# VISION-SJTU/UniDefense

Measured on AMD Instinct MI355X. Metric: images/sec fwd+bwd (256x256, EffNet-b4), higher is better.
Workload: dtype f32

## Files before the change

include/unidefense_hip.h:

```cpp
#ifndef UNIDEFENSE_HIP_H
#define UNIDEFENSE_HIP_H
#include <stdint.h>

#ifdef __cplusplus
extern "C" {
#endif

#define UD_EINVAL (-1000)

typedef void* ud_stream_t;

typedef struct {
    int N, Hin, Win, Cin, Hout, Wout, KH, KW, stride, pad_t, pad_l, transposed;
} ud_conv_geom;

typedef struct {
    const float* A; const float* B; float* C;
    int M, N, K;
    long lda, ldb, ldc;
    int a_mode, b_mode, out_mode, split_k;
    int batch; long strideA, strideB, strideC;
    ud_conv_geom g;
    double* stat_sum; double* stat_sumsq;
    int half_mask;
    int tile_cfg;
    long slice_stride;
} ud_gemm_desc;
int ud_gemm(const ud_gemm_desc* d, ud_stream_t stream);
int ud_sum_slices(const float* ws, float* out, int slices, long total, long slice_stride, int accumulate,
                  ud_stream_t stream);
int ud_gemm_stats_slots(const ud_gemm_desc* d);
int ud_stat_slots_fold(const double* slot_sum, const double* slot_sumsq, int slots, int N, double* acc_sum,
                       double* acc_sumsq, ud_stream_t stream);
int ud_gemm_set_path(int path);
int ud_gemm_get_path(void);
int ud_gemm_query_path(const ud_gemm_desc* d);

typedef struct {
    const uint16_t* A; const uint16_t* B; float* C;
    int M, N, K;
    long a_panel, a_plane, b_panel, b_plane;
    int a_npanel, b_npanel;
    long ldc;
    int a_mode, b_mode, out_mode, split_k;
    double* stat_sum; double* stat_sumsq;
    int tile_cfg;
    long slice_stride;
    int prec;
    const float* a_inv_scale; const float* b_inv_scale;
    int a_scale_stride, b_scale_stride;
    int c_half;
} ud_gemm_p3_desc;
int ud_gemm_p3(const ud_gemm_p3_desc* d, ud_stream_t stream);
int ud_gemm_p3_pair(const ud_gemm_p3_desc* nn, const ud_gemm_p3_desc* tn, ud_stream_t stream);
int ud_planes_from_half(const void* x, long R, int C, long ld, uint16_t* planes, long panel_stride, float* inv_scale,
                        ud_stream_t stream);
int ud_split_planes(const float* x, long R, int C, long ld, uint16_t* planes, long panel_stride, long plane_stride,
                    ud_stream_t stream);
int ud_split_planes_h2(const float* x, long R, int C, long ld, uint16_t* planes, long panel_stride, long plane_stride,
                       float* inv_scale, ud_stream_t stream);
int ud_absmax(const float* x, long R, int C, long ld, uint32_t* absmax, ud_stream_t stream);
int ud_split_planes_h2t(const float* x, long R, int C, long ld, uint16_t* planes, long panel_stride, long plane_stride,
                        const uint32_t* absmax, float* inv_scale, ud_stream_t stream);
typedef struct {
    const float* x; uint16_t* out; float* inv_scale;
    long R, ld, panel, plane;
    int C, amax_block0, amax_blocks, split_block0, split_bx, pad_;
} ud_split_item;
int ud_split_planes_h2t_multi(const ud_split_item* items_dev, int n, uint32_t* slots, int amax_blocks_total,
                              int split_blocks_total, ud_stream_t stream);

int ud_im2col_planes(const float* x, const ud_conv_geom* g, uint16_t* planes, long panel_stride, long plane_stride,
                     const uint32_t* absmax, float* inv_scale, ud_stream_t stream);
int ud_col2im(const float* dcol, const ud_conv_geom* g, float* dx, ud_stream_t stream);

typedef struct {
    const float* src;
    float* dst;
    int A, B, KH, KW, mode, block0;
} ud_layout_item;
int ud_weight_layouts_multi(const ud_layout_item* items_dev, int n, int blocks_total, ud_stream_t stream);

int ud_reduce_ws_doubles(int G, int R, int C);
int ud_norm_stats(const float* x, int G, int R, int C, float eps, double* ws, float* mean, float* invstd,
                  float* var_out, float momentum, float* running_mean, float* running_var, ud_stream_t stream);
int ud_syncbn_combine(const float* gathered, int world, int C, long rows_per_rank, float eps, float momentum,
                      float* running_mean, float* running_var, float* mean, float* invstd, ud_stream_t stream);
int ud_norm_apply_fwd(const float* x, int G, int R, int C, const float* mean, const float* invstd,
                      const float* gamma, const float* beta, int act, float* y, ud_stream_t stream);
int ud_norm_bwd(const float* x, const float* dy, int G, int R, int C, const float* mean, const float* invstd,
                const float* gamma, const float* beta, int act, double* ws, float* s1, float* s2, float* dgamma,
                float* dbeta, float* dx, ud_stream_t stream);
int ud_norm_bwd_apply(const float* x, const float* dy, int G, int R, int C, const float* mean,
                      const float* invstd, const float* gamma, const float* beta, const float* s1,
                      const float* s2, float inv_count, int act, float* dx, ud_stream_t stream);
int ud_group_colsum(const float* x, int G, int R, int C, float scale, double* ws, float* out, ud_stream_t stream);
int ud_group_coldot(const float* a, const float* b, int G, int R, int C, float scale, double* ws, float* out,
                    ud_stream_t stream);
int ud_bcast_rows(const float* g, float scale, float* out, int N, int HW, int C, ud_stream_t stream);

int ud_dwconv_fwd(const void* x, const float* wt, void* y, int N, int H, int W, int C, int Ho, int Wo, int K,
    int stride, int pad_t, int pad_l, int f16, ud_stream_t stream);
int ud_dwconv_bwd_data(const void* dy, const float* wt, const void* add, void* dx, int N, int H, int W, int C,
    int Ho, int Wo, int K, int stride, int pad_t, int pad_l, int f16, ud_stream_t stream);
int ud_dwconv_bwd_weight_parts(int C, int chunks);
int ud_dw_weights_tapmajor(const void* table, int layers, long max_elems, float* dst, ud_stream_t stream);
int ud_dwconv_bwd_weight(const float* x, const float* dy, float* dwt, float* part, int chunks, int N,
// ... 543 lines not shown
```

unidefense_amd/csrc/gemm_p3.hip:

```cpp
#include "gemm_internal.h"
#include "ud_common.h"

#include <algorithm>
#include <type_traits>

namespace {

constexpr int NT = 512;
constexpr int BK = 32;
constexpr int BM = 128, BN = 128;
constexpr int PLANE_IMG = 128 * 64;

template <int PREC> struct Cfg {
    static constexpr int NPL = PREC;
    static constexpr int OP_IMG = NPL * PLANE_IMG;
    static constexpr int STAGE = 2 * OP_IMG;
    static constexpr int NSTAGE = PREC == 3 ? 3 : 4;
    static constexpr int PT = 4 * NPL;
    static constexpr int NTERM = PREC == 3 ? 6 : PREC == 2 ? 3 : 1;
};

typedef __bf16 bf16x8 __attribute__((ext_vector_type(8)));
typedef _Float16 f16x8 __attribute__((ext_vector_type(8)));
typedef short s16x4 __attribute__((ext_vector_type(4)));
typedef short s16x8 __attribute__((ext_vector_type(8)));
typedef __attribute__((address_space(3))) char lds_char;

__device__ __forceinline__ void dma_piece(unsigned voff, unsigned lds_dst, const char* gbase) {
    unsigned keep;
    asm volatile(
        "s_nop 1\n\t"
        "s_mov_b32 %0, m0\n\t"
        "s_mov_b32 m0, %2\n\t"
        "s_nop 0\n\t"
        "global_load_lds_dwordx4 %1, %3\n\t"
        "s_mov_b32 m0, %0"
        : "=&s"(keep)
        : "v"(voff), "s"(lds_dst), "s"(gbase));
}

template <int N>
__device__ __forceinline__ void wait_dma_and_barrier() {
    asm volatile("s_waitcnt vmcnt(%0) lgkmcnt(0)\n\ts_barrier" ::"n"(N) : "memory");
}
template <int PT>
__device__ __forceinline__ void wait_tiles_and_barrier(int tiles) {
    if (tiles <= 0) wait_dma_and_barrier<0>();
    else if (tiles == 1) wait_dma_and_barrier<PT>();
    else if (tiles == 2) wait_dma_and_barrier<2 * PT>();
    else if (tiles == 3 || PT > 4) wait_dma_and_barrier<3 * PT>();
    else if (tiles == 4) wait_dma_and_barrier<4 * PT>();
    else if (tiles == 5) wait_dma_and_barrier<5 * PT>();
    else wait_dma_and_barrier<6 * PT>();
// ... 23 lines not shown
    }

    template <int S, int I, int PL, int NPL>
    __device__ __forceinline__ void read_one(const lds_char* img, Frags<NPL>& f) const {
        if constexpr (MODE == 0) {
            const lds_char* p = img + (S == 0 ? b0 : b1) + I * 2048 + PL * PLANE_IMG;
            f.v[I][PL] = *reinterpret_cast<const __attribute__((address_space(3))) s16x8*>(p);
        } else {
            const lds_char* p = img + b0 + S * 1024 + I * 2048 + PL * PLANE_IMG;
            const s16x4 lo = __builtin_amdgcn_ds_read_tr16_b64_v4i16((__attribute__((address_space(3))) s16x4*)(p));
            const s16x4 hi = __builtin_amdgcn_ds_read_tr16_b64_v4i16((__attribute__((address_space(3))) s16x4*)(p + 256));
            f.v[I][PL] = __builtin_shufflevector(lo, hi, 0, 1, 2, 3, 4, 5, 6, 7);
        }
    }

    template <int S, int NPL>
    __device__ __forceinline__ void read(const lds_char* img, Frags<NPL>& f) const {
        read_one<S, 0, 0>(img, f); read_one<S, 1, 0>(img, f);
        if constexpr (NPL >= 2) { read_one<S, 0, 1>(img, f); read_one<S, 1, 1>(img, f); }
        if constexpr (NPL == 3) { read_one<S, 0, 2>(img, f); read_one<S, 1, 2>(img, f); }
    }
};

template <int MODE>
__device__ __forceinline__ unsigned dma_lane_offset(int lane) {
    if constexpr (MODE == 0) return (unsigned)((lane >> 2) * 64 + (((lane & 3) ^ ((lane >> 4) & 3)) << 4));
    else return (unsigned)(lane * 16);
}

template <int PREC, int TERM> struct Term {
    static constexpr int pa = PREC == 3 ? (TERM == 0 ? 2 : (TERM == 1 || TERM >= 4) ? 0 : 1) : PREC == 2 ? (TERM == 0 ? 1 : 0) : 0;
    static constexpr int pb = PREC == 3 ? (TERM == 0 ? 0 : TERM == 1 ? 2 : (TERM == 2 || TERM == 4) ? 1 : 0) : PREC == 2 ? (TERM == 1 ? 1 : 0) : 0;
};

template <int PREC, int Mi>
__device__ __forceinline__ void mma_one(f32x16 (&acc)[2][2], f32x16 (&lo)[2][2], const Frags<PREC>& a, const Frags<PREC>& b) {
    constexpr int term = Mi / 4, i = (Mi % 4) / 2, j = Mi % 2;
    using Tm = Term<PREC, term>;
    if constexpr (PREC == 3) {
        acc[i][j] = __builtin_amdgcn_mfma_f32_32x32x16_bf16(__builtin_bit_cast(bf16x8, a.v[i][Tm::pa]),
                                                            __builtin_bit_cast(bf16x8, b.v[j][Tm::pb]), acc[i][j], 0, 0, 0);
    } else if constexpr (PREC == 1) {
        acc[i][j] = __builtin_amdgcn_mfma_f32_32x32x16_f16(__builtin_bit_cast(f16x8, a.v[i][0]),
                                                           __builtin_bit_cast(f16x8, b.v[j][0]), acc[i][j], 0, 0, 0);
    } else if constexpr (term < 2) {
        lo[i][j] = __builtin_amdgcn_mfma_f32_32x32x16_f16(__builtin_bit_cast(f16x8, a.v[i][Tm::pa]),
                                                          __builtin_bit_cast(f16x8, b.v[j][Tm::pb]), lo[i][j], 0, 0, 0);
    } else {
        acc[i][j] = __builtin_amdgcn_mfma_f32_32x32x16_f16(__builtin_bit_cast(f16x8, a.v[i][Tm::pa]),
                                                           __builtin_bit_cast(f16x8, b.v[j][Tm::pb]), acc[i][j], 0, 0, 0);
    }
}

template <int PREC, int AMODE, int BMODE, bool SK>
__device__ __forceinline__ void p3_body(const ud_gemm_p3_desc& d, int tiles_m, int tiles_n, char* L, int bx, int by, int gx) {
    using CF = Cfg<PREC>;
    constexpr int NPL = CF::NPL, OP_IMG = CF::OP_IMG, STAGE = CF::STAGE, NSTAGE = CF::NSTAGE, PT = CF::PT;

    const int tid = threadIdx.x, lane = tid & 63;
    const int wave = __builtin_amdgcn_readfirstlane(tid >> 6);
    const int wm = (wave >> 1) & 1, wn = wave & 1;
    const int l31 = lane & 31, half = lane >> 5;
    const int kt_total = d.K / BK;
    const int dM = d.M, dN = d.N;
    const long ldc = d.ldc;
    const bool c_half = d.c_half != 0;
    double* const stat_sum = d.stat_sum;
    double* const stat_sumsq = d.stat_sumsq;
    const float* const a_inv = d.a_inv_scale;
    const float* const b_inv = d.b_inv_scale;
    const long ast = d.a_scale_stride, bst = d.b_scale_stride;
    const lds_char* Lp = (const lds_char*)L;
    const unsigned lds0 = (unsigned)(uintptr_t)Lp;
    const int lw = wave & 3;
    const unsigned dst_w = lds0 + (unsigned)lw * 2048u;
    const long a_plane = d.a_plane * 2, b_plane = d.b_plane * 2;
    const unsigned a_voff = dma_lane_offset<AMODE>(lane), b_voff = dma_lane_offset<BMODE>(lane);
    Reader<AMODE> ra;
    Reader<BMODE> rb;
    ra.init(lane, wm * 64);
    rb.init(lane, wn * 64);
    using std::integral_constant;
    using H0 = integral_constant<int, 0>;
    using H1 = integral_constant<int, 1>;
    using T = std::true_type;
    using F = std::false_type;

    auto segment = [&](int tile_m, int tile_n, int kt0, int nkt, int ep, float* Cp, bool first) {
        const int m0 = tile_m * BM, n0 = tile_n * BN;
        f32x16 acc[2][2], lo[PREC == 2 ? 2 : 1][2];
#pragma unroll
        for (int i = 0; i < 2; ++i)
#pragma unroll
            for (int j = 0; j < 2; ++j)
#pragma unroll
                for (int r = 0; r < 16; ++r) {
                    acc[i][j][r] = 0.f;
                    if constexpr (PREC == 2) lo[i][j][r] = 0.f;
                }

        if (nkt > 0) {
            if (wave >= 4) {
                const char* a_g0;
                const char* b_g0;
                long a_step, b_step;
                if constexpr (AMODE == 0) {
                    a_g0 = reinterpret_cast<const char*>(d.A) + (long)kt0 * d.a_panel * 2 + (long)(m0 + 32 * lw) * 64;
                    a_step = d.a_panel * 2;
                } else {
                    a_g0 = reinterpret_cast<const char*>(d.A) + (long)min(m0 / 32 + lw, d.a_npanel - 1) * d.a_panel * 2 +
                           (long)kt0 * BK * 64;
                    a_step = BK * 64;
                }
                if constexpr (BMODE == 0) {
                    b_g0 = reinterpret_cast<const char*>(d.B) + (long)kt0 * d.b_panel * 2 + (long)(n0 + 32 * lw) * 64;
                    b_step = d.b_panel * 2;
                } else {
                    b_g0 = reinterpret_cast<const char*>(d.B) + (long)min(n0 / 32 + lw, d.b_npanel - 1) * d.b_panel * 2 +
                           (long)kt0 * BK * 64;
                    b_step = BK * 64;
                }
                auto issue = [&](int t) {
                    const unsigned dst = dst_w + (unsigned)(t % NSTAGE) * STAGE;
                    const char* ga = a_g0 + (long)t * a_step;
                    const char* gb = b_g0 + (long)t * b_step;
#pragma unroll
                    for (int pl = 0; pl < NPL; ++pl)
#pragma unroll
                        for (int jj = 0; jj < 2; ++jj)
                            dma_piece(a_voff, dst + pl * PLANE_IMG + jj * 1024, ga + pl * a_plane + jj * 1024);
#pragma unroll
                    for (int pl = 0; pl < NPL; ++pl)
#pragma unroll
                        for (int jj = 0; jj < 2; ++jj)
                            dma_piece(b_voff, dst + OP_IMG + pl * PLANE_IMG + jj * 1024, gb + pl * b_plane + jj * 1024);
                };
                if (!first) wait_dma_and_barrier<0>();
                const int pro = min(nkt, NSTAGE);
                for (int t = 0; t < pro; ++t) issue(t);
                wait_tiles_and_barrier<PT>(pro - 1);
                for (int t = 0; t + 1 < nkt; ++t) {
                    wait_tiles_and_barrier<PT>(min(nkt, t + NSTAGE) - (t + 2));
                    if (t + NSTAGE < nkt) issue(t + NSTAGE);
                }
                return;
            }
            if (!first) wait_lds_and_barrier();
            wait_lds_and_barrier();

            f32x16 (&lo2)[2][2] = *reinterpret_cast<f32x16 (*)[2][2]>(&lo[0][0]);
            Frags<NPL> fa0, fb0, fa1, fb1;
            ra.template read<0>(Lp, fa0);
            rb.template read<0>(Lp + OP_IMG, fb0);

            auto phase = [&](auto rs_c, auto do_read_c, const Frags<NPL>& ca, const Frags<NPL>& cb, Frags<NPL>& na, Frags<NPL>& nb,
                             const lds_char* img) {
                constexpr int RS = decltype(rs_c)::value;
                constexpr bool RD = decltype(do_read_c)::value;
                constexpr int NSLOT = 2 * NPL, PER = 4 * CF::NTERM / NSLOT;
                auto slot = [&](auto k_c) {
                    constexpr int k = decltype(k_c)::value;
                    constexpr int ai = k & 1, bi = k & 1;
                    constexpr int apl = NPL == 3 ? (k < 2 ? 2 : k < 4 ? 0 : 1) : NPL == 2 ? (k < 2 ? 1 : 0) : 0;
                    constexpr int bpl = NPL == 3 ? (k < 2 ? 0 : k < 4 ? 2 : 1) : NPL == 2 ? (k < 2 ? 0 : 1) : 0;
                    if constexpr (RD) {
                        ra.template read_one<RS, ai, apl>(img, na);
                        rb.template read_one<RS, bi, bpl>(img + OP_IMG, nb);
                    }
                    mma_one<PREC, PER * k>(acc, lo2, ca, cb);
                    mma_one<PREC, PER * k + 1>(acc, lo2, ca, cb);
                    if constexpr (PER >= 3) mma_one<PREC, PER * k + 2>(acc, lo2, ca, cb);
                    if constexpr (PER == 4) mma_one<PREC, PER * k + 3>(acc, lo2, ca, cb);
                    __builtin_amdgcn_sched_barrier(0);
                };
                slot(integral_constant<int, 0>{}); slot(integral_constant<int, 1>{});
                if constexpr (NSLOT >= 4) { slot(integral_constant<int, 2>{}); slot(integral_constant<int, 3>{}); }
                if constexpr (NSLOT == 6) { slot(integral_constant<int, 4>{}); slot(integral_constant<int, 5>{}); }
            };
            for (int t = 0; t + 1 < nkt; ++t) {
                phase(H1{}, T{}, fa0, fb0, fa1, fb1, Lp + (t % NSTAGE) * STAGE);
                wait_lds_and_barrier();
                phase(H0{}, T{}, fa1, fb1, fa0, fb0, Lp + ((t + 1) % NSTAGE) * STAGE);
            }
            phase(H1{}, T{}, fa0, fb0, fa1, fb1, Lp + ((nkt - 1) % NSTAGE) * STAGE);
            phase(H0{}, F{}, fa1, fb1, fa0, fb0, Lp);
        } else if (wave >= 4) {
            return;
        }

        if (nkt <= 0 && ep != 0) return;
        if constexpr (PREC <= 2) {
            const float* __restrict__ as = a_inv;
            const float* __restrict__ bs = b_inv;
            float ib[2], ia[2][16];
#pragma unroll
            for (int j = 0; j < 2; ++j) ib[j] = bs[(long)min(n0 + wn * 64 + j * 32 + l31, dN - 1) * bst];
            if (ast == 0) {
                const float a0 = as[0];
#pragma unroll
                for (int i = 0; i < 2; ++i)
#pragma unroll
                    for (int r = 0; r < 16; ++r) ia[i][r] = a0;
            } else {
#pragma unroll
                for (int i = 0; i < 2; ++i)
#pragma unroll
                    for (int r = 0; r < 16; ++r)
                        ia[i][r] = as[min(m0 + wm * 64 + i * 32 + (r & 3) + 8 * (r >> 2) + 4 * half, dM - 1)];
            }
#pragma unroll
            for (int j = 0; j < 2; ++j) {
                const bool cok = n0 + wn * 64 + j * 32 + l31 < dN;
#pragma unroll
                for (int i = 0; i < 2; ++i)
#pragma unroll
                    for (int r = 0; r < 16; ++r) {
                        const int row = m0 + wm * 64 + i * 32 + (r & 3) + 8 * (r >> 2) + 4 * half;
                        float v = acc[i][j][r];
                        if constexpr (PREC == 2) v += 0x1p-11f * lo[i][j][r];
                        v *= ia[i][r] * ib[j];
                        asm volatile("" : "+v"(v));
                        acc[i][j][r] = (cok && row < dM) ? v : 0.f;
                    }
            }
        }
        if (!SK && stat_sum) {
            if (PREC == 3 && m0 + BM > dM) {
#pragma unroll
                for (int i = 0; i < 2; ++i)
#pragma unroll
                    for (int r = 0; r < 16; ++r) {
                        const int row = m0 + wm * 64 + i * 32 + (r & 3) + 8 * (r >> 2) + 4 * half;
                        if (row >= dM) { acc[i][0][r] = 0.f; acc[i][1][r] = 0.f; }
                    }
            }
            const long slot = (tiles_m > 64) ? (long)(tile_m & 63) * dN : 0;
#pragma unroll
            for (int j = 0; j < 2; ++j) {
                double s1 = 0.0, s2 = 0.0;
// ... 13 lines not shown
                    unsafeAtomicAdd(stat_sumsq + slot + col, s2);
                }
            }
        }
        auto store_all = [&](auto mode_c, auto inside_c) {
            constexpr int MODE = decltype(mode_c)::value;
            constexpr bool INSIDE = decltype(inside_c)::value;
#pragma unroll
            for (int i = 0; i < 2; ++i) {
#pragma unroll
                for (int j = 0; j < 2; ++j) {
                    const int col = n0 + wn * 64 + j * 32 + l31;
                    const long off0 = (long)(m0 + wm * 64 + i * 32 + 4 * half) * ldc + col;
                    float* pc = Cp + off0;
#pragma unroll
                    for (int r = 0; r < 16; ++r) {
                        const int dr = (r & 3) + 8 * (r >> 2);
                        if (INSIDE || (m0 + wm * 64 + i * 32 + 4 * half + dr < dM && col < dN)) {
                            const float v = acc[i][j][r];
                            if constexpr (MODE >= 4) {
                                _Float16* p = reinterpret_cast<_Float16*>(Cp) + off0 + (long)dr * ldc;
                                *p = (_Float16)(MODE == 4 ? v : v + (float)*p);
                            } else {
                                float* p = pc + (long)dr * ldc;
                                if constexpr (MODE == 0) *p = v;
                                else if constexpr (MODE == 1) *p += v;
                                else atomicAdd(p, v);
                            }
                        }
                    }
                }
            }
        };
        const bool inside = m0 + BM <= dM && n0 + BN <= dN;
        if (PREC == 1 && c_half) {
            if (inside) {
                if (ep == 0) store_all(integral_constant<int, 4>{}, T{});
                else store_all(integral_constant<int, 5>{}, T{});
            } else {
                if (ep == 0) store_all(integral_constant<int, 4>{}, F{});
                else store_all(integral_constant<int, 5>{}, F{});
            }
        } else if (inside) {
            if (ep == 0) store_all(integral_constant<int, 0>{}, T{});
            else if (ep == 1) store_all(integral_constant<int, 1>{}, T{});
            else store_all(integral_constant<int, 2>{}, T{});
        } else {
            if (ep == 0) store_all(integral_constant<int, 0>{}, F{});
            else if (ep == 1) store_all(integral_constant<int, 1>{}, F{});
            else store_all(integral_constant<int, 2>{}, F{});
        }
    };

    if constexpr (!SK) {
        int tile_m = bx % tiles_m, tile_n = bx / tiles_m;
        if (d.tile_cfg & 0x200) {
            const int GM = (d.tile_cfg >> 12) & 15 ? (d.tile_cfg >> 12) & 15 : 4;
            const int Tn = tiles_m * tiles_n, q = Tn >> 3, r = Tn & 7, x = bx & 7;
            const int o = x * q + (x < r ? x : r) + (bx >> 3);
            const int per_group = GM * tiles_n, g = o / per_group, first_m = g * GM;
            const int gm = min(GM, tiles_m - first_m), in = o - g * per_group;
            tile_n = in / gm;
            tile_m = first_m + in - tile_n * gm;
        }
        const int split = by;
        const int kt_per = (kt_total + d.split_k - 1) / d.split_k;
        const int kt0 = split * kt_per;
        const int nkt = min(kt_per, kt_total - kt0);
        segment(tile_m, tile_n, kt0, nkt, d.out_mode == 3 ? 0 : d.out_mode,
                d.C + (d.out_mode == 3 ? (long)split * d.slice_stride : 0L), true);
    } else {
        const int G = gx, b = bx;
        const int g = (b & 7) * (G >> 3) + (b >> 3);
        const long U = (long)tiles_m * tiles_n * kt_total;
        long u = g * U / G;
        const long u1 = (g + 1) * U / G;
        const int band_tiles = 8 * tiles_m;
        bool first = true;
        while (u < u1) {
            const int tile = (int)(u / kt_total), kt_b = (int)(u - (long)tile * kt_total);
            const int kt_e = (int)min((long)kt_total, kt_b + (u1 - u));
            const int band = tile / band_tiles, in_band = tile - band * band_tiles;
            const int bw = min(8, tiles_n - band * 8);
            const int tile_m = in_band / bw, tile_n = band * 8 + in_band - tile_m * bw;
            const bool whole = kt_b == 0 && kt_e == kt_total;
            segment(tile_m, tile_n, kt_b, kt_e - kt_b, whole ? d.out_mode : 2, d.C, first);
            first = false;
            u += kt_e - kt_b;
        }
    }
}

template <int PREC, int AMODE, int BMODE, bool SK = false>
__global__ __launch_bounds__(NT, 1) void gemm_p3_kernel(const ud_gemm_p3_desc d, int tiles_m, int tiles_n) {
    using CF = Cfg<PREC>;
    __shared__ __attribute__((aligned(1024))) char L[CF::NSTAGE * CF::STAGE];
    p3_body<PREC, AMODE, BMODE, SK>(d, tiles_m, tiles_n, L, (int)blockIdx.x, (int)blockIdx.y, (int)gridDim.x);
}

template <int PREC, int A0 = 0, int B0 = 1, int A1 = 1, int B1 = 1>
__global__ __launch_bounds__(NT, 1) void gemm_p3_pair_kernel(const ud_gemm_p3_desc d0, int tm0, int tn0, int n0,
                                                              const ud_gemm_p3_desc d1, int tm1, int tn1) {
    using CF = Cfg<PREC>;
    __shared__ __attribute__((aligned(1024))) char L[CF::NSTAGE * CF::STAGE];
    const int b = (int)blockIdx.x;
    const bool first = b < (n0 < 0 ? -n0 : n0);
    const int l = first ? b : b - (n0 < 0 ? -n0 : n0);
    if (first == (n0 > 0)) {
        const int T = tm0 * tn0;
        p3_body<PREC, A0, B0, false>(d0, tm0, tn0, L, l % T, l / T, T);
    } else {
        const int T = tm1 * tn1;
        p3_body<PREC, A1, B1, false>(d1, tm1, tn1, L, l % T, l / T, T);
    }
}

int num_cus() {
    static const int n = [] {
        int dev = 0, cus = 0;
        if (hipGetDevice(&dev) != hipSuccess ||
            hipDeviceGetAttribute(&cus, hipDeviceAttributeMultiprocessorCount, dev) != hipSuccess || cus < 8)
            cus = 256;
        return cus;
    }();
    return n;
}

template <int PREC, int AMODE, int BMODE>
int launch(const ud_gemm_p3_desc& d, hipStream_t s) {
    const int tiles_m = ud_cdiv(d.M, BM), tiles_n = ud_cdiv(d.N, BN);
    if (d.tile_cfg & 0x800) {
        const long U = (long)tiles_m * tiles_n * (d.K / BK);
        long G = std::min<long>(num_cus(), U / 4);
        G = std::max<long>(8, G / 8 * 8);
        hipLaunchKernelGGL((gemm_p3_kernel<PREC, AMODE, BMODE, true>), dim3((unsigned)G), dim3(NT), 0, s, d, tiles_m, tiles_n);
    } else {
        dim3 grid((unsigned)(tiles_m * tiles_n), (unsigned)d.split_k, 1);
        hipLaunchKernelGGL((gemm_p3_kernel<PREC, AMODE, BMODE>), grid, dim3(NT), 0, s, d, tiles_m, tiles_n);
    }
    UD_LAUNCH_CHECK();
    return 0;
}

__device__ __forceinline__ uint32_t pack_bf16(float x, float y) {
    typedef __bf16 bf16x2 __attribute__((ext_vector_type(2)));
    bf16x2 v = {(__bf16)x, (__bf16)y};
    return __builtin_bit_cast(uint32_t, v);
}
__device__ __forceinline__ void split2(float x, float y, uint32_t& p0, uint32_t& p1, uint32_t& p2) {
    p0 = pack_bf16(x, y);
    const float rx = x - __uint_as_float(p0 << 16), ry = y - __uint_as_float(p0 & 0xffff0000u);
    p1 = pack_bf16(rx, ry);
    const float sx = rx - __uint_as_float(p1 << 16), sy = ry - __uint_as_float(p1 & 0xffff0000u);
    p2 = pack_bf16(sx, sy);
}

typedef uint32_t u32x4 __attribute__((ext_vector_type(4)));
typedef uint32_t u32x2 __attribute__((ext_vector_type(2)));

__global__ __launch_bounds__(256) void split_planes_kernel(const float* __restrict__ x, long R, int C, long ld,
                                                           uint16_t* __restrict__ out, long panel, long plane) {
    const int tid = threadIdx.x;
    const long row = (long)blockIdx.x * 64 + (tid >> 2);
    const int pan = blockIdx.y, c0 = pan * 32 + (tid & 3) * 8;
    if (row >= R) return;
    f32x4 v0 = {0.f, 0.f, 0.f, 0.f}, v1 = {0.f, 0.f, 0.f, 0.f};
    if (c0 + 8 <= C) {
        v0 = *reinterpret_cast<const f32x4*>(x + row * ld + c0);
        v1 = *reinterpret_cast<const f32x4*>(x + row * ld + c0 + 4);
    } else if (c0 + 4 <= C) {
        v0 = *reinterpret_cast<const f32x4*>(x + row * ld + c0);
    }
    uint32_t a[4], b[4], c[4];
    split2(v0[0], v0[1], a[0], b[0], c[0]);
    split2(v0[2], v0[3], a[1], b[1], c[1]);
    split2(v1[0], v1[1], a[2], b[2], c[2]);
    split2(v1[2], v1[3], a[3], b[3], c[3]);
    const u32x4 p0 = {a[0], a[1], a[2], a[3]}, p1 = {b[0], b[1], b[2], b[3]}, p2 = {c[0], c[1], c[2], c[3]};
    uint16_t* o = out + (long)pan * panel + row * 32 + (tid & 3) * 8;
    *reinterpret_cast<u32x4*>(o) = p0;
    *reinterpret_cast<u32x4*>(o + plane) = p1;
    *reinterpret_cast<u32x4*>(o + 2 * plane) = p2;
}
// ... 321 lines not shown
    return 0;
}

extern "C" int ud_planes_from_half(const void* x, long R, int C, long ld, uint16_t* planes, long panel_stride, float* inv_scale,
                                   ud_stream_t stream) {
    if (!x || !planes || !inv_scale || R < 1 || C < 8 || C % 8 || ld < C || ld % 8 || panel_stride < 32 * R || panel_stride % 8 ||
        ((uintptr_t)x & 15))
        return UD_EINVAL;
    dim3 grid((unsigned)ud_cdiv(R, 64), (unsigned)ud_cdiv(C, 32));
    hipLaunchKernelGGL(planes_from_half_kernel, grid, dim3(256), 0, (hipStream_t)stream, (const uint16_t*)x, R, C, ld, planes,
                       panel_stride, inv_scale);
    UD_LAUNCH_CHECK();
    return 0;
}

extern "C" int ud_split_planes(const float* x, long R, int C, long ld, uint16_t* planes, long panel_stride,
                               long plane_stride, ud_stream_t stream) {
    if (!x || !planes || R <= 0 || C <= 0 || C % 4 != 0 || ld % 4 != 0 || ld < C || panel_stride < R * 32 ||
        panel_stride % 8 != 0 || plane_stride % 8 != 0 || plane_stride < (long)ud_cdiv(C, 32) * panel_stride)
        return UD_EINVAL;
    dim3 grid((unsigned)ud_cdiv(R, 64), (unsigned)ud_cdiv(C, 32));
    hipLaunchKernelGGL(split_planes_kernel, grid, dim3(256), 0, (hipStream_t)stream, x, R, C, ld, planes, panel_stride,
                       plane_stride);
    UD_LAUNCH_CHECK();
    return 0;
}

extern "C" int ud_split_planes_h2(const float* x, long R, int C, long ld, uint16_t* planes, long panel_stride,
                                  long plane_stride, float* inv_scale, ud_stream_t stream) {
    if (!x || !planes || !inv_scale || R <= 0 || C <= 0 || C % 4 != 0 || C > 256 * H2_MAXQ || ld % 4 != 0 || ld < C ||
        panel_stride < R * 32 || panel_stride % 8 != 0 || plane_stride % 8 != 0 ||
        plane_stride < (long)ud_cdiv(C, 32) * panel_stride)
        return UD_EINVAL;
    hipLaunchKernelGGL(split_h2_rows_kernel, dim3((unsigned)ud_cdiv(R, 4)), dim3(256), 0, (hipStream_t)stream, x, R, C, ld,
                       planes, panel_stride, plane_stride, inv_scale);
    UD_LAUNCH_CHECK();
    return 0;
}

static bool p3_desc_ok(const ud_gemm_p3_desc& d);

extern "C" int ud_gemm_p3_pair(const ud_gemm_p3_desc* nn, const ud_gemm_p3_desc* tn, ud_stream_t stream) {
    if (!nn || !tn || !p3_desc_ok(*nn) || !p3_desc_ok(*tn)) return UD_EINVAL;
    const ud_gemm_p3_desc &d0 = *nn, &d1 = *tn;
    const bool grads = d0.a_mode == 0 && d0.b_mode == 1 && d1.a_mode == 1 && d1.b_mode == 1;
    const bool tailp = d0.a_mode == 0 && d0.b_mode == 0 && d1.a_mode == 0 && d1.b_mode == 0 && d0.prec == 2;
    if ((d0.prec != 2 && d0.prec != 1) || d1.prec != d0.prec || !(grads || tailp)) return UD_EINVAL;
    if ((d0.tile_cfg | d1.tile_cfg) & 0x800) return UD_EINVAL;
    if (d0.stat_sum || d1.stat_sum || d0.out_mode == 3 || d1.out_mode == 3) return UD_EINVAL;
    const int tm0 = ud_cdiv(d0.M, BM), tn0 = ud_cdiv(d0.N, BN), tm1 = ud_cdiv(d1.M, BM), tn1 = ud_cdiv(d1.N, BN);
    const long n0 = (long)tm0 * tn0 * d0.split_k, n1 = (long)tm1 * tn1 * d1.split_k;
    if (n0 + n1 > 0x7fffffffL) return UD_EINVAL;
    const int nfirst = (d1.tile_cfg & 0x10000) ? -(int)n1 : (int)n0;
    if (tailp)
        hipLaunchKernelGGL((gemm_p3_pair_kernel<2, 0, 0, 0, 0>), dim3((unsigned)(n0 + n1)), dim3(NT), 0, (hipStream_t)stream, d0, tm0,
                           tn0, nfirst, d1, tm1, tn1);
    else if (d0.prec == 1)
        hipLaunchKernelGGL((gemm_p3_pair_kernel<1>), dim3((unsigned)(n0 + n1)), dim3(NT), 0, (hipStream_t)stream, d0, tm0, tn0,
                           nfirst, d1, tm1, tn1);
    else
        hipLaunchKernelGGL((gemm_p3_pair_kernel<2>), dim3((unsigned)(n0 + n1)), dim3(NT), 0, (hipStream_t)stream, d0, tm0, tn0,
                           nfirst, d1, tm1, tn1);
    UD_LAUNCH_CHECK();
    return 0;
}

static bool p3_desc_ok(const ud_gemm_p3_desc& d) {
    if (!d.A || !d.B || !d.C || d.M <= 0 || d.N <= 0 || d.K <= 0 || d.K % BK != 0 || d.split_k < 1 ||
        d.split_k > d.K / BK || d.out_mode < 0 || d.out_mode > 3 || d.a_mode < 0 || d.a_mode > 1 || d.b_mode < 0 ||
        d.b_mode > 1 || d.a_panel % 8 != 0 || d.b_panel % 8 != 0 || d.a_plane % 8 != 0 || d.b_plane % 8 != 0 ||
        d.a_npanel < 1 || d.b_npanel < 1 || d.prec < 1 || d.prec > 3)
        return false;
    if (d.prec <= 2 && (!d.a_inv_scale || !d.b_inv_scale || d.a_scale_stride < 0 || d.a_scale_stride > 1 ||
                        d.b_scale_stride < 0 || d.b_scale_stride > 1))
        return false;
    if (d.stat_sum && (d.out_mode != 0 || d.split_k != 1 || !d.stat_sumsq || (d.tile_cfg & 0x800))) return false;
    if ((d.tile_cfg & 0x800) && (d.out_mode > 1 || d.split_k != 1)) return false;
    if (d.out_mode == 3 && d.slice_stride < (long)d.M * d.ldc) return false;
    if (d.c_half && (d.prec != 1 || d.out_mode > 1 || d.split_k != 1 || (d.tile_cfg & 0x800))) return false;
    return true;
}

extern "C" int ud_gemm_p3(const ud_gemm_p3_desc* dp, ud_stream_t stream) {
    if (!dp) return UD_EINVAL;
    const ud_gemm_p3_desc& d = *dp;
    if (!p3_desc_ok(d)) return UD_EINVAL;
    hipStream_t s = (hipStream_t)stream;
    if (d.prec == 1) {
        if (d.a_mode == 0 && d.b_mode == 0) return launch<1, 0, 0>(d, s);
        if (d.a_mode == 0 && d.b_mode == 1) return launch<1, 0, 1>(d, s);
        if (d.a_mode == 1 && d.b_mode == 1) return launch<1, 1, 1>(d, s);
        return UD_EINVAL;
    }
    if (d.prec == 2) {
        if (d.a_mode == 0 && d.b_mode == 0) return launch<2, 0, 0>(d, s);
        if (d.a_mode == 0 && d.b_mode == 1) return launch<2, 0, 1>(d, s);
        if (d.a_mode == 1 && d.b_mode == 1) return launch<2, 1, 1>(d, s);
        return UD_EINVAL;
    }
    if (d.a_mode == 0 && d.b_mode == 0) return launch<3, 0, 0>(d, s);
    if (d.a_mode == 0 && d.b_mode == 1) return launch<3, 0, 1>(d, s);
    if (d.a_mode == 1 && d.b_mode == 1) return launch<3, 1, 1>(d, s);
    if (d.a_mode == 1 && d.b_mode == 0) return launch<3, 1, 0>(d, s);
    return UD_EINVAL;
}
```

unidefense_amd/kernels.py:

```python
import contextlib
import ctypes as C
import math
import os

import torch

from . import lib as _lib
from .config import cfg as CFG
from .devmem import Scratch, ZeroPool
from .lib import ConvGeom, GemmDesc, GemmP3Desc

_call = _lib.call
_const, _rows = _lib.const, _lib.const_rows

GEMM_PROFILE = None


def _stream():
    return C.c_void_p(torch.cuda.current_stream().cuda_stream)


def _p(t):
    if t is None:
        return None
# ... 320 lines not shown
    if mode == 1:
        return w.flip(2, 3).permute(1, 2, 3, 0).reshape(B, KH * KW * A).contiguous()
    return w.permute(1, 2, 3, 0).reshape(B, KH * KW * A).contiguous()


def begin_forward(owner=None):
    global _WEIGHT_PLANES, _WEIGHT_LAYOUTS
    reset_zero_pool()
    if owner is not None:
        batch = owner.__dict__.get("_ud_weight_planes")
        if batch is None:
            batch = owner.__dict__["_ud_weight_planes"] = _WeightPlaneBatch()
        _WEIGHT_PLANES = batch
        lay = owner.__dict__.get("_ud_weight_layouts")
        if lay is None:
            lay = owner.__dict__["_ud_weight_layouts"] = _WeightLayoutBatch()
        _WEIGHT_LAYOUTS = lay
    _WEIGHT_PLANES.begin()
    _WEIGHT_LAYOUTS.begin()


def end_forward():
    _WEIGHT_PLANES.active = False
    _WEIGHT_LAYOUTS.active = False


def weight_batch_snapshot():
    return [(b, {k: e[2] for k, e in b.entries.items()}) for b in (_WEIGHT_PLANES, _WEIGHT_LAYOUTS)]


def weight_batch_check(snapshot):
    for b, versions in snapshot:
        for k, v in versions.items():
            e = b.entries.get(k)
            if e is not None and v >= 0 and e[2] >= 0 and e[2] != v:
                raise RuntimeError("backward of a forward whose weight planes / layouts have been re-made from updated weights "
                                   "by a later forward (forward A, optimizer step, forward B, backward A): run A's backward first")


def weight_planes(w2):
    pl = _WEIGHT_PLANES.lookup(w2)
    if pl is not None:
        return pl
    _WEIGHT_PLANES.register(w2)
    return split_planes(w2, prec=2)


def p3_ok(M, N, K):
    return K % 32 == 0 and min(M, N) >= 128 and K >= 128


_P3_RASTER = 0x4200
_P3_STAT_SLOT_TILES = 64


def _p3_desc(A, B, Cout, M, N, K, a_mode, b_mode, out_mode=0, split_k=1, a_row0=0, cfg=0):
    d = GemmP3Desc()
    if a_mode == 0:
        d.A = A.buf.data_ptr() + 2 * (a_row0 * 32)
        d.a_npanel = A.npanel
    else:
        d.A = A.buf.data_ptr() + 2 * ((a_row0 // 32) * A.panel)
        d.a_npanel = A.npanel - a_row0 // 32
    d.B = B.buf.data_ptr()
    d.b_npanel = B.npanel
    d.C = Cout.data_ptr()
    d.M, d.N, d.K = M, N, K
    d.a_panel, d.a_plane, d.b_panel, d.b_plane = A.panel, A.plane, B.panel, B.plane
    d.ldc = N
    d.a_mode, d.b_mode, d.out_mode, d.split_k = a_mode, b_mode, out_mode, split_k
    d.tile_cfg = cfg | (_P3_RASTER if not cfg & 0x800 else 0)
    assert A.prec == B.prec or max(A.prec, B.prec) <= 2
    d.prec = min(A.prec, B.prec)
    d.c_half = 1 if Cout.dtype == torch.float16 else 0
    if d.prec <= 2:
        assert (a_mode == 0 or not A.scale_stride) and (b_mode == 0 or not B.scale_stride)
        d.a_inv_scale = A.inv.data_ptr() + 4 * a_row0 * A.scale_stride
        d.b_inv_scale = B.inv.data_ptr()
        d.a_scale_stride, d.b_scale_stride = A.scale_stride, B.scale_stride
    return d


_P3_PAIR = True


def _p3_pair_tn_first(M, N, Kd, pn, pt):
    sp = int(pt[1]) if pt[0] == "split" else 1
    t1 = -(-N // 128) * -(-Kd // 128) * sp
    return M / sp > 2.0 * N and t1 <= 256


def _p3_pair_ok(pn, pt):
    return pn[0] in ("plain", "split", "sk") and pt[0] in ("plain", "split")


def spectral_bwd(ctx, dy2, out=None, dy_absmax=None):
    if (ctx.plans is None or not _P3_PAIR or CFG.deterministic or GEMM_PROFILE is not None or
            not _p3_pair_ok(ctx.plans["nn"], ctx.plans["tn"])):
        dw = spectral_wgrad(ctx, dy2, dy_absmax)
        return spectral_dgrad(ctx, dy2, out=out, dy_absmax=dy_absmax), dw
    dy = _spectral_dy(ctx, dy2, dy_absmax)
    pn, pt = ctx.plans["nn"], ctx.plans["tn"]
    if pn[0] == "sk":
        pn = ("plain",)
    M, N, Kd = ctx.M, ctx.N, ctx.K
    acc = out is not None
    if pn[0] == "plain":
        dx = out if acc else empty((M, Kd), dy2, torch.float16 if dy2.dtype == torch.float16 else torch.float32)
        d0 = _p3_desc(dy, ctx.w, dx, M, Kd, -(-N // 32) * 32, 0, 1, 1 if acc else 0, 1)
    else:
        dx = out if acc else split_out((M, Kd), dy2)
        d0 = _p3_desc(dy, ctx.w, dx, M, Kd, -(-N // 32) * 32, 0, 1, 2, int(pn[1]))
    if pt[0] == "plain":
        dw = empty((N, Kd), dy2)
        d1 = _p3_desc(dy, ctx.x, dw, N, Kd, -(-M // 32) * 32, 1, 1, 0, 1)
    else:
        dw = split_out((N, Kd), dy2)
        d1 = _p3_desc(dy, ctx.x, dw, N, Kd, -(-M // 32) * 32, 1, 1, 2, int(pt[1]))
    if _p3_pair_tn_first(M, N, Kd, pn, pt):
        d1.tile_cfg |= 0x10000
    _call("ud_gemm_p3_pair", C.byref(d0), C.byref(d1), _stream())
    return dx, dw


def _gemm_p3(A, B, Cout, M, N, K, a_mode, b_mode, out_mode=0, split_k=1, stats=None, a_row0=0, cfg=0):
    d = _p3_desc(A, B, Cout, M, N, K, a_mode, b_mode, out_mode, split_k, a_row0, cfg)
    slices = None
    if CFG.deterministic and out_mode == 2:
        total = M * N
        fresh = getattr(Cout, "_ud_fresh", False)
        ws = _slice_ws(Cout, split_k * total)
        d.C, d.out_mode, d.slice_stride = ws.data_ptr(), 3, total
        slices = (ws, total, total, 0 if fresh else 1)
        if fresh:
            Cout._ud_fresh = False
    fold = None
    stats_done = False
    if stats is not None and out_mode == 0 and split_k == 1:
        stats_done = True
        slots = 64 if -(-M // 128) > _P3_STAT_SLOT_TILES else 1
        tgt = stats if slots == 1 else zeros64(2 * slots * N, Cout)
        d.stat_sum, d.stat_sumsq = tgt.data_ptr(), tgt.data_ptr() + 8 * (slots * N if slots > 1 else N)
        if slots > 1:
            fold = (tgt, slots)
    if GEMM_PROFILE is not None:
        e0, e1 = torch.cuda.Event(enable_timing=True), torch.cuda.Event(enable_timing=True)
        e0.record()
        _call("ud_gemm_p3", C.byref(d), _stream())
        e1.record()
        GEMM_PROFILE.append((e0, e1, 2.0 * M * N * K, (M, N, K, a_mode, b_mode, split_k, 1), 4,
                             2.0 * A.prec * (M * K + K * N) + 4.0 * M * N))
    else:
        _call("ud_gemm_p3", C.byref(d), _stream())
    if slices is not None:
        ws, stride, total, accumulate = slices
        _call("ud_sum_slices", _p(ws), _p(Cout), split_k, total, stride, accumulate, _stream())
    if fold is not None:
        tgt, slots = fold
        _call("ud_stat_slots_fold", _pd64(tgt), _pd64(tgt, slots * N), slots, N, _pd64(stats), _pd64(stats, N), _stream())
    return (Cout, stats_done) if stats is not None else Cout


_TAIL_SPLIT = True


def _pd64(t, off_doubles=0):
    return C.c_void_p(t.data_ptr() + 8 * off_doubles)


def _tail_plan(M, N, K):
    if not _TAIL_SPLIT or M < 1024 or N < 128 or K < 512:
        return None
    mt, nt = -(-M // 128), -(-N // 128)
# ... 3238 lines not shown
```

Baseline: 1451.

## Add persistent-worker P3 GEMM kernel with streaming loader across tile units

Adds a persistent kernel for the two-plane (PREC==2) P3 GEMM. A fixed number of workgroups (defaulting to the CU count) loops over tile/split-k units, and a dedicated loader wave group streams DMA loads across unit boundaries so the LDS pipeline stays full between tiles. It is enabled by default for single GEMMs when there are more units than workers. The backward pair path is left off by a flag. This aims to cut per-workgroup launch and prologue/epilogue pipeline bubbles, at the cost of more complex cross-unit stage bookkeeping and possible load imbalance from static round-robin assignment.

```diff
diff --git a/include/unidefense_hip.h b/include/unidefense_hip.h
--- a/include/unidefense_hip.h
+++ b/include/unidefense_hip.h
@@ -53,6 +53,7 @@
 } ud_gemm_p3_desc;
 int ud_gemm_p3(const ud_gemm_p3_desc* d, ud_stream_t stream);
 int ud_gemm_p3_pair(const ud_gemm_p3_desc* nn, const ud_gemm_p3_desc* tn, ud_stream_t stream);
+int ud_gemm_p3_units(const ud_gemm_p3_desc* d0, const ud_gemm_p3_desc* d1, int workers, int worker, int* out, int cap);
 int ud_planes_from_half(const void* x, long R, int C, long ld, uint16_t* planes, long panel_stride, float* inv_scale,
                         ud_stream_t stream);
 int ud_split_planes(const float* x, long R, int C, long ld, uint16_t* planes, long panel_stride, long plane_stride,
diff --git a/unidefense_amd/csrc/gemm_p3.hip b/unidefense_amd/csrc/gemm_p3.hip
--- a/unidefense_amd/csrc/gemm_p3.hip
+++ b/unidefense_amd/csrc/gemm_p3.hip
@@ -1,4 +1,5 @@
 #include "gemm_internal.h"
+#include "gemm_p3_units.h"
 #include "ud_common.h"
 
 #include <algorithm>
@@ -128,8 +129,9 @@
     }
 }
 
-template <int PREC, int AMODE, int BMODE, bool SK>
-__device__ __forceinline__ void p3_body(const ud_gemm_p3_desc& d, int tiles_m, int tiles_n, char* L, int bx, int by, int gx) {
+template <int PREC, int AMODE, int BMODE, bool SK, bool PS = false>
+__device__ __forceinline__ void p3_body(const ud_gemm_p3_desc& d, int tiles_m, int tiles_n, char* L, int bx, int by, int gx,
+                                        const P3Unit* pu = nullptr, int s0 = 0, bool fresh = true) {
     using CF = Cfg<PREC>;
     constexpr int NPL = CF::NPL, OP_IMG = CF::OP_IMG, STAGE = CF::STAGE, NSTAGE = CF::NSTAGE, PT = CF::PT;
 
@@ -175,8 +177,9 @@
                     if constexpr (PREC == 2) lo[i][j][r] = 0.f;
                 }
 
+        const int sb = PS ? s0 : 0;
         if (nkt > 0) {
-            if (wave >= 4) {
+            if (!PS && wave >= 4) {
                 const char* a_g0;
                 const char* b_g0;
                 long a_step, b_step;
@@ -221,13 +224,17 @@
                 }
                 return;
             }
-            if (!first) wait_lds_and_barrier();
-            wait_lds_and_barrier();
+            if constexpr (PS) {
+                if (first) wait_lds_and_barrier();
+            } else {
+                if (!first) wait_lds_and_barrier();
+                wait_lds_and_barrier();
+            }
 
             f32x16 (&lo2)[2][2] = *reinterpret_cast<f32x16 (*)[2][2]>(&lo[0][0]);
             Frags<NPL> fa0, fb0, fa1, fb1;
-            ra.template read<0>(Lp, fa0);
-            rb.template read<0>(Lp + OP_IMG, fb0);
+            ra.template read<0>(Lp + (sb % NSTAGE) * STAGE, fa0);
+            rb.template read<0>(Lp + (sb % NSTAGE) * STAGE + OP_IMG, fb0);
 
             auto phase = [&](auto rs_c, auto do_read_c, const Frags<NPL>& ca, const Frags<NPL>& cb, Frags<NPL>& na, Frags<NPL>& nb,
                              const lds_char* img) {
@@ -254,13 +261,14 @@
                 if constexpr (NSLOT == 6) { slot(integral_constant<int, 4>{}); slot(integral_constant<int, 5>{}); }
             };
             for (int t = 0; t + 1 < nkt; ++t) {
-                phase(H1{}, T{}, fa0, fb0, fa1, fb1, Lp + (t % NSTAGE) * STAGE);
+                phase(H1{}, T{}, fa0, fb0, fa1, fb1, Lp + ((sb + t) % NSTAGE) * STAGE);
                 wait_lds_and_barrier();
-                phase(H0{}, T{}, fa1, fb1, fa0, fb0, Lp + ((t + 1) % NSTAGE) * STAGE);
+                phase(H0{}, T{}, fa1, fb1, fa0, fb0, Lp + ((sb + t + 1) % NSTAGE) * STAGE);
             }
-            phase(H1{}, T{}, fa0, fb0, fa1, fb1, Lp + ((nkt - 1) % NSTAGE) * STAGE);
+            phase(H1{}, T{}, fa0, fb0, fa1, fb1, Lp + ((sb + nkt - 1) % NSTAGE) * STAGE);
+            if constexpr (PS) wait_lds_and_barrier();
             phase(H0{}, F{}, fa1, fb1, fa0, fb0, Lp);
-        } else if (wave >= 4) {
+        } else if (!PS && wave >= 4) {
             return;
         }
 
@@ -380,17 +388,12 @@
         }
     };
 
-    if constexpr (!SK) {
-        int tile_m = bx % tiles_m, tile_n = bx / tiles_m;
-        if (d.tile_cfg & 0x200) {
-            const int GM = (d.tile_cfg >> 12) & 15 ? (d.tile_cfg >> 12) & 15 : 4;
-            const int Tn = tiles_m * tiles_n, q = Tn >> 3, r = Tn & 7, x = bx & 7;
-            const int o = x * q + (x < r ? x : r) + (bx >> 3);
-            const int per_group = GM * tiles_n, g = o / per_group, first_m = g * GM;
-            const int gm = min(GM, tiles_m - first_m), in = o - g * per_group;
-            tile_n = in / gm;
-            tile_m = first_m + in - tile_n * gm;
-        }
+    if constexpr (PS) {
+        segment(pu->tile_m, pu->tile_n, pu->kt0, pu->nkt, d.out_mode == 3 ? 0 : d.out_mode,
+                d.C + (d.out_mode == 3 ? (long)pu->split * d.slice_stride : 0L), fresh);
+    } else if constexpr (!SK) {
+        int tile_m, tile_n;
+        p3_tile_of(tiles_m, tiles_n, d.tile_cfg, bx, tile_m, tile_n);
         const int split = by;
         const int kt_per = (kt_total + d.split_k - 1) / d.split_k;
         const int kt0 = split * kt_per;
@@ -443,6 +446,117 @@
     }
 }
 
+struct P3Src {
+    const char* a_g0;
+    const char* b_g0;
+    long a_step, b_step;
+    long a_plane, b_plane;
+    bool a_m1, b_m1;
+};
+
+template <int AMODE, int BMODE>
+__device__ __forceinline__ P3Src p3_src_of(const ud_gemm_p3_desc& d, const P3Unit& u, int lw) {
+    P3Src r;
+    const int m0 = u.tile_m * BM, n0 = u.tile_n * BN;
+    if constexpr (AMODE == 0) {
+        r.a_g0 = reinterpret_cast<const char*>(d.A) + (long)u.kt0 * d.a_panel * 2 + (long)(m0 + 32 * lw) * 64;
+        r.a_step = d.a_panel * 2;
+    } else {
+        r.a_g0 = reinterpret_cast<const char*>(d.A) + (long)min(m0 / 32 + lw, d.a_npanel - 1) * d.a_panel * 2 + (long)u.kt0 * BK * 64;
+        r.a_step = BK * 64;
+    }
+    if constexpr (BMODE == 0) {
+        r.b_g0 = reinterpret_cast<const char*>(d.B) + (long)u.kt0 * d.b_panel * 2 + (long)(n0 + 32 * lw) * 64;
+        r.b_step = d.b_panel * 2;
+    } else {
+        r.b_g0 = reinterpret_cast<const char*>(d.B) + (long)min(n0 / 32 + lw, d.b_npanel - 1) * d.b_panel * 2 + (long)u.kt0 * BK * 64;
+        r.b_step = BK * 64;
+    }
+    r.a_plane = d.a_plane * 2;
+    r.b_plane = d.b_plane * 2;
+    r.a_m1 = AMODE == 1;
+    r.b_m1 = BMODE == 1;
+    return r;
+}
+
+template <int PREC, int A0, int B0, int A1, int B1, bool PAIR>
+__device__ __forceinline__ void p3_loader_stream(const ud_gemm_p3_desc& d0, const ud_gemm_p3_desc& d1, const P3Sched& sc, char* L,
+                                                 int w, int W) {
+    using CF = Cfg<PREC>;
+    constexpr int NPL = CF::NPL, OP_IMG = CF::OP_IMG, STAGE = CF::STAGE, NSTAGE = CF::NSTAGE, PT = CF::PT;
+    const int lane = threadIdx.x & 63;
+    const int lw = __builtin_amdgcn_readfirstlane(threadIdx.x >> 6) & 3;
+    const unsigned dst_w = (unsigned)(uintptr_t)(const lds_char*)L + (unsigned)lw * 2048u;
+    const unsigned voff0 = dma_lane_offset<0>(lane), voff1 = dma_lane_offset<1>(lane);
+
+    int u_next = w, t = 0, nkt = 0;
+    P3Src src;
+    auto open_next = [&]() -> bool {
+        while (u_next < sc.n_units) {
+            const P3Unit u = p3_unit(sc, u_next);
+            u_next += W;
+            if (u.nkt <= 0) continue;
+            if (!PAIR || u.prob == 0) src = p3_src_of<A0, B0>(d0, u, lw);
+            else src = p3_src_of<A1, B1>(d1, u, lw);
+            t = 0;
+            nkt = u.nkt;
+            return true;
+        }
+        return false;
+    };
+    bool have = open_next();
+    int st = 0, issued = 0;
+    if (have) {
+        auto issue = [&]() {
+            const unsigned dst = dst_w + (unsigned)st * STAGE;
+            const char* ga = src.a_g0 + (long)t * src.a_step;
+            const char* gb = src.b_g0 + (long)t * src.b_step;
+            const unsigned a_voff = src.a_m1 ? voff1 : voff0, b_voff = src.b_m1 ? voff1 : voff0;
+#pragma unroll
+            for (int pl = 0; pl < NPL; ++pl)
+#pragma unroll
+                for (int jj = 0; jj < 2; ++jj) dma_piece(a_voff, dst + pl * PLANE_IMG + jj * 1024, ga + pl * src.a_plane + jj * 1024);
+#pragma unroll
+            for (int pl = 0; pl < NPL; ++pl)
+#pragma unroll
+                for (int jj = 0; jj < 2; ++jj)
+                    dma_piece(b_voff, dst + OP_IMG + pl * PLANE_IMG + jj * 1024, gb + pl * src.b_plane + jj * 1024);
+            st = st + 1 == NSTAGE ? 0 : st + 1;
+            ++issued;
+            if (++t == nkt) have = open_next();
+        };
+        while (have && issued < NSTAGE) issue();
+        wait_tiles_and_barrier<PT>(issued - 1);
+        for (int s = 0; s < issued; ++s) {
+            wait_tiles_and_barrier<PT>(issued - (s + 2));
+            if (have) issue();
+        }
+    }
+}
+
+template <int PREC, int A0, int B0, int A1, int B1, bool PAIR>
+__global__ __launch_bounds__(NT, 1) void gemm_p3_persist_kernel(const ud_gemm_p3_desc d0, const ud_gemm_p3_desc d1, const P3Sched sc) {
+    using CF = Cfg<PREC>;
+    __shared__ __attribute__((aligned(1024))) char L[CF::NSTAGE * CF::STAGE];
+    const int wave = __builtin_amdgcn_readfirstlane(threadIdx.x >> 6);
+    const int w = (int)blockIdx.x, W = (int)gridDim.x;
+    if (wave >= 4) {
+        p3_loader_stream<PREC, A0, B0, A1, B1, PAIR>(d0, d1, sc, L, w, W);
+        return;
+    }
+    int s0 = 0;
+    bool fresh = true;
+    for (int i = w; i < sc.n_units; i += W) {
+        const P3Unit u = p3_unit(sc, i);
+        if (!PAIR || u.prob == 0) p3_body<PREC, A0, B0, false, true>(d0, sc.p0.tiles_m, sc.p0.tiles_n, L, 0, 0, 0, &u, s0, fresh);
+        else p3_body<PREC, A1, B1, false, true>(d1, sc.p1.tiles_m, sc.p1.tiles_n, L, 0, 0, 0, &u, s0, fresh);
+        if (u.nkt > 0) {
+            s0 = (s0 + u.nkt) % CF::NSTAGE;
+            fresh = false;
+        }
+    }
+}
+
 int num_cus() {
     static const int n = [] {
         int dev = 0, cus = 0;
@@ -454,9 +568,24 @@
     return n;
 }
 
+int persist_workers(int tile_cfg, long n_units) {
+    if (tile_cfg & P3_CFG_ONE_UNIT) return 0;
+    const int W = p3_cfg_workers(tile_cfg) ? p3_cfg_workers(tile_cfg) : num_cus();
+    return n_units > W ? W : 0;
+}
+
 template <int PREC, int AMODE, int BMODE>
 int launch(const ud_gemm_p3_desc& d, hipStream_t s) {
     const int tiles_m = ud_cdiv(d.M, BM), tiles_n = ud_cdiv(d.N, BN);
+    if constexpr (PREC == 2) {
+        const P3Sched sc = p3_sched_of(d, nullptr);
+        if (const int W = (d.tile_cfg & 0x800) ? 0 : persist_workers(d.tile_cfg, sc.n_units)) {
+            hipLaunchKernelGGL((gemm_p3_persist_kernel<2, AMODE, BMODE, AMODE, BMODE, false>), dim3((unsigned)W), dim3(NT), 0, s, d, d,
+                               sc);
+            UD_LAUNCH_CHECK();
+            return 0;
+        }
+    }
     if (d.tile_cfg & 0x800) {
         const long U = (long)tiles_m * tiles_n * (d.K / BK);
         long G = std::min<long>(num_cus(), U / 4);
@@ -884,6 +1013,17 @@
     const long n0 = (long)tm0 * tn0 * d0.split_k, n1 = (long)tm1 * tn1 * d1.split_k;
     if (n0 + n1 > 0x7fffffffL) return UD_EINVAL;
     const int nfirst = (d1.tile_cfg & 0x10000) ? -(int)n1 : (int)n0;
+    if (const int W = d0.prec == 2 ? persist_workers(d0.tile_cfg, n0 + n1) : 0) {
+        const P3Sched sc = p3_sched_of(d0, &d1);
+        if (tailp)
+            hipLaunchKernelGGL((gemm_p3_persist_kernel<2, 0, 0, 0, 0, true>), dim3((unsigned)W), dim3(NT), 0, (hipStream_t)stream, d0, d1,
+                               sc);
+        else
+            hipLaunchKernelGGL((gemm_p3_persist_kernel<2, 0, 1, 1, 1, true>), dim3((unsigned)W), dim3(NT), 0, (hipStream_t)stream, d0, d1,
+                               sc);
+        UD_LAUNCH_CHECK();
+        return 0;
+    }
     if (tailp)
         hipLaunchKernelGGL((gemm_p3_pair_kernel<2, 0, 0, 0, 0>), dim3((unsigned)(n0 + n1)), dim3(NT), 0, (hipStream_t)stream, d0, tm0,
                            tn0, nfirst, d1, tm1, tn1);
@@ -913,6 +1053,24 @@
     return true;
 }
 
+extern "C" int ud_gemm_p3_units(const ud_gemm_p3_desc* d0, const ud_gemm_p3_desc* d1, int workers, int worker, int* out, int cap) {
+    auto geom_ok = [](const ud_gemm_p3_desc* d) {
+        return d->M > 0 && d->N > 0 && d->K > 0 && d->K % BK == 0 && d->split_k >= 1 && d->split_k <= d->K / BK;
+    };
+    if (!d0 || !geom_ok(d0) || (d1 && !geom_ok(d1)) || workers < 1 || worker < 0 || worker >= workers || cap < 0 || (cap && !out))
+        return UD_EINVAL;
+    if (p3_prob_units(p3_prob_of(*d0)) + (d1 ? p3_prob_units(p3_prob_of(*d1)) : 0) > 0x7fffffffL) return UD_EINVAL;
+    const P3Sched sc = p3_sched_of(*d0, d1);
+    int n = 0;
+    for (long i = worker; i < sc.n_units; i += workers, ++n)
+        if (n < cap) {
+            const P3Unit u = p3_unit(sc, (int)i);
+            const int v[8] = {u.prob, u.tile_m, u.tile_n, u.split, u.kt0, u.nkt, u.bar_loader, u.bar_mfma};
+            std::copy(v, v + 8, out + 8 * (long)n);
+        }
+    return n;
+}
+
 extern "C" int ud_gemm_p3(const ud_gemm_p3_desc* dp, ud_stream_t stream) {
     if (!dp) return UD_EINVAL;
     const ud_gemm_p3_desc& d = *dp;
diff --git a/unidefense_amd/csrc/gemm_p3_units.h b/unidefense_amd/csrc/gemm_p3_units.h
--- /dev/null
+++ b/unidefense_amd/csrc/gemm_p3_units.h
@@ -0,0 +1,79 @@
+#pragma once
+#include "../../include/unidefense_hip.h"
+
+#if defined(__HIPCC__) || defined(__CUDACC__)
+#define UD_P3_HD __host__ __device__ __forceinline__
+#else
+#define UD_P3_HD inline
+#endif
+
+constexpr int P3_BK = 32, P3_BM = 128, P3_BN = 128;
+
+constexpr int P3_CFG_RASTER = 0x200, P3_CFG_ONE_UNIT = 0x20000;
+UD_P3_HD int p3_cfg_workers(int tile_cfg) { return (tile_cfg >> 20) & 0x3ff; }
+
+struct P3Unit {
+    int prob, tile_m, tile_n, split, kt0, nkt;
+    int bar_loader, bar_mfma;
+};
+struct P3Prob {
+    int tiles_m, tiles_n, split_k, kt_total, tile_cfg;
+};
+struct P3Sched {
+    P3Prob p0, p1;
+    int lead;
+    int n_lead, n_units;
+};
+
+UD_P3_HD long p3_prob_units(const P3Prob& q) { return (long)q.tiles_m * q.tiles_n * q.split_k; }
+
+UD_P3_HD void p3_tile_of(int tiles_m, int tiles_n, int tile_cfg, int bx, int& tile_m, int& tile_n) {
+    tile_m = bx % tiles_m;
+    tile_n = bx / tiles_m;
+    if (tile_cfg & P3_CFG_RASTER) {
+        const int GM = (tile_cfg >> 12) & 15 ? (tile_cfg >> 12) & 15 : 4;
+        const int Tn = tiles_m * tiles_n, q = Tn >> 3, r = Tn & 7, x = bx & 7;
+        const int o = x * q + (x < r ? x : r) + (bx >> 3);
+        const int per_group = GM * tiles_n, g = o / per_group, first_m = g * GM;
+        const int gm = GM < tiles_m - first_m ? GM : tiles_m - first_m, in = o - g * per_group;
+        tile_n = in / gm;
+        tile_m = first_m + in - tile_n * gm;
+    }
+}
+
+UD_P3_HD int p3_unit_barriers_loader(int nkt) { return nkt > 0 ? nkt : 0; }
+UD_P3_HD int p3_unit_barriers_mfma(int nkt) { return nkt > 0 ? (nkt - 1) + 1 : 0; }
+
+UD_P3_HD P3Unit p3_unit(const P3Sched& sc, int idx) {
+    const bool lead = idx < sc.n_lead;
+    const int prob = lead ? sc.lead : 1 - sc.lead, l = lead ? idx : idx - sc.n_lead;
+    const int tiles_m = prob ? sc.p1.tiles_m : sc.p0.tiles_m, tiles_n = prob ? sc.p1.tiles_n : sc.p0.tiles_n;
+    const int split_k = prob ? sc.p1.split_k : sc.p0.split_k, kt_total = prob ? sc.p1.kt_total : sc.p0.kt_total;
+    const int tile_cfg = prob ? sc.p1.tile_cfg : sc.p0.tile_cfg;
+    const int T = tiles_m * tiles_n;
+    P3Unit u;
+    u.prob = prob;
+    u.split = l / T;
+    p3_tile_of(tiles_m, tiles_n, tile_cfg, l - u.split * T, u.tile_m, u.tile_n);
+    const int kt_per = (kt_total + split_k - 1) / split_k;
+    u.kt0 = u.split * kt_per;
+    const int left = kt_total - u.kt0;
+    u.nkt = left < 0 ? 0 : left < kt_per ? left : kt_per;
+    u.bar_loader = p3_unit_barriers_loader(u.nkt);
+    u.bar_mfma = p3_unit_barriers_mfma(u.nkt);
+    return u;
+}
+
+inline P3Prob p3_prob_of(const ud_gemm_p3_desc& d) {
+    return P3Prob{(d.M + P3_BM - 1) / P3_BM, (d.N + P3_BN - 1) / P3_BN, d.split_k, d.K / P3_BK, d.tile_cfg};
+}
+inline P3Sched p3_sched_of(const ud_gemm_p3_desc& d0, const ud_gemm_p3_desc* d1) {
+    P3Sched sc;
+    sc.p0 = p3_prob_of(d0);
+    sc.p1 = d1 ? p3_prob_of(*d1) : sc.p0;
+    sc.lead = d1 && (d1->tile_cfg & 0x10000) ? 1 : 0;
+    const long n0 = p3_prob_units(sc.p0), n1 = d1 ? p3_prob_units(sc.p1) : 0;
+    sc.n_lead = (int)(sc.lead ? n1 : n0);
+    sc.n_units = (int)(n0 + n1);
+    return sc;
+}
diff --git a/unidefense_amd/kernels.py b/unidefense_amd/kernels.py
--- a/unidefense_amd/kernels.py
+++ b/unidefense_amd/kernels.py
@@ -396,6 +396,14 @@
 
 _P3_RASTER = 0x4200
 _P3_STAT_SLOT_TILES = 64
+_P3_PERSIST = True
+_P3_PERSIST_GRADS = False
+_P3_WORKERS = 0
+
+
+def _p3_persist_cfg(on=True):
+    assert 0 <= _P3_WORKERS < 1024
+    return (0 if _P3_PERSIST and on else 0x20000) | (_P3_WORKERS << 20)
 
 
 def _p3_desc(A, B, Cout, M, N, K, a_mode, b_mode, out_mode=0, split_k=1, a_row0=0, cfg=0):
@@ -413,7 +421,7 @@
     d.a_panel, d.a_plane, d.b_panel, d.b_plane = A.panel, A.plane, B.panel, B.plane
     d.ldc = N
     d.a_mode, d.b_mode, d.out_mode, d.split_k = a_mode, b_mode, out_mode, split_k
-    d.tile_cfg = cfg | (_P3_RASTER if not cfg & 0x800 else 0)
+    d.tile_cfg = cfg | (_P3_RASTER if not cfg & 0x800 else 0) | _p3_persist_cfg()
     assert A.prec == B.prec or max(A.prec, B.prec) <= 2
     d.prec = min(A.prec, B.prec)
     d.c_half = 1 if Cout.dtype == torch.float16 else 0
@@ -463,6 +471,7 @@
         d1 = _p3_desc(dy, ctx.x, dw, N, Kd, -(-M // 32) * 32, 1, 1, 2, int(pt[1]))
     if _p3_pair_tn_first(M, N, Kd, pn, pt):
         d1.tile_cfg |= 0x10000
+    d0.tile_cfg |= _p3_persist_cfg(_P3_PERSIST_GRADS) & 0x20000
     _call("ud_gemm_p3_pair", C.byref(d0), C.byref(d1), _stream())
     return dx, dw
 
```

New measurement: 1451, median of 2. Within noise of the previous version (+0.0%).
